# johannes-graeter/limo

Hardware: AMD Instinct MI355X
Metric: keyframe-BA window solves/sec (5 KF, ~2k landmarks) (higher is better)
Workload: dtype f64; 1 GPU; C2: KITTI-00-shaped windows, 5 keyframes x 2000 landmarks, LiDAR depth + ground plane, solveTrimmed schedule {2, trim 5%, <=100 LM iterations}; batch_windows_per_gpu=16384, distinct_windows_per_gpu=4096, observations_per_batch=144288124, depth_observations_per_batch=68405568, parallelism=single, converged=16328

## Files before the change

### limo_amd/csrc/kba_buffers.hpp

```cpp
#pragma once
#include <algorithm>
#include <cstddef>
#include <vector>

#include "kba_pack.hpp"

namespace kba {

template <typename F>
void for_each_buffer(const PackedBatch& P, BatchView& bv, F f) {
    bv.n_win = P.n_win;
    bv.TK = P.TK;
    bv.TL = P.TL;
    bv.TO = P.TO;
    bv.TV = P.TV;
    bv.TG = P.TG;
    bv.n_blk = P.n_blk;
    bv.n_lblk = P.n_lblk;
    bv.n_sblk = P.n_sblk;
    bv.Vmax = P.Vmax;
    bv.SO = P.SO;
    bv.SL = P.SL;
    bv.SG = P.SG;
    bv.SD = P.SD;
// ... 19 lines not shown
    KBA_BUF(lm_c, TL * 3 * D, P.lm.data());
    KBA_BUF(kf_win, TK * I, P.kf_win.data());
    KBA_BUF(kf_blk0, TK * I, P.kf_blk0.data());
    KBA_BUF(kf_nblk, TK * I, P.kf_nblk.data());
    KBA_BUF(kf_gp0, TK * I, P.kf_gp0.data());
    KBA_BUF(kf_ngp, TK * I, P.kf_ngp.data());
    KBA_BUF(cmask, TK * kCamSlots, P.cmask.data());
    KBA_BUF(cpresent, TK * kCamSlots, P.cpresent.data());
    KBA_BUF(cslot, TK * kCamSlots * I, P.cslot.data());
    KBA_BUF(lm_win, TL * I, P.lm_win.data());
    KBA_BUF(lm_id, TL * I, P.lm_id.data());
    KBA_BUF(lm_weight, TL * D, P.lm_weight.data());
    KBA_BUF(lm_state, TL, P.lm_state.data());
    KBA_BUF(lm_gp, TL * I, P.lm_gp.data());
    KBA_BUF(lm_slot, P.lm_slot.size() * I, P.lm_slot.data());
    KBA_BUF(view_kf, TV * I, P.view_kf.data());
    KBA_BUF(view_win, TV * I, P.view_win.data());
    KBA_BUF(view_cam, TV * 16 * D, P.view_cam.data());
    KBA_BUF(view_lin, TV * kViewLin * D, nullptr);
    KBA_BUF(view_lin_c, TV * kViewLin * D, nullptr);
    KBA_BUF(blk_view, NB * I, P.blk_view.data());
    KBA_BUF(blk_obs0, NB * I, P.blk_obs0.data());
    KBA_BUF(blk_n, NB * I, P.blk_n.data());
    KBA_BUF(obs_lm, TO * I, P.obs_lm.data());
    KBA_BUF(obs_u, TO * sizeof(float), P.obs_u.data());
    KBA_BUF(obs_v, TO * sizeof(float), P.obs_v.data());
    KBA_BUF(obs_d, TO * sizeof(float), P.obs_d.data());
    KBA_BUF(lblk_win, NL * I, P.lblk_win.data());
    KBA_BUF(lblk_lm0, NL * I, P.lblk_lm0.data());
    KBA_BUF(lblk_n, NL * I, P.lblk_n.data());
    KBA_BUF(sblk_win, NS * I, P.sblk_win.data());
    KBA_BUF(sblk_lm0, NS * I, P.sblk_lm0.data());
    KBA_BUF(sblk_n, NS * I, P.sblk_n.data());
    KBA_BUF(gp_lm, TG * I, P.gp_lm.data());
    KBA_BUF(gp_kf, TG * I, P.gp_kf.data());
    KBA_BUF(gp_w, TG * D, P.gp_w.data());
    KBA_BUF(gp_r, (size_t)P.SG * D, nullptr);
    KBA_BUF(gp_F, (size_t)P.SG * 10 * D, nullptr);
    KBA_BUF(gp_E, (size_t)P.SG * 3 * D, nullptr);
    KBA_BUF(gp_cost, TG * D, nullptr);
    KBA_BUF(gp_cost_c, TG * D, nullptr);
    KBA_BUF(obs_r, (size_t)(P.evaluate_only ? P.SO * 2 + P.SD : 1) * D, nullptr);
    KBA_BUF(obs_c, (size_t)(P.evaluate_only ? 1 : P.SO * 2) * D, nullptr);
    KBA_BUF(obs_Jp, (size_t)(P.evaluate_only ? P.SO * 12 + P.SD * 6 : 1) * D, nullptr);
    KBA_BUF(obs_Jl, (size_t)(P.evaluate_only ? P.SO * 6 + P.SD * 3 : 1) * D, nullptr);
    if (P.evaluate_only) KBA_BUF(echunk, (size_t)std::max(1, P.n_echunk) * sizeof(EvalChunk), P.echunk.empty() ? nullptr : P.echunk.data());
    KBA_BUF(lv_part, (size_t)(P.lvpart_total > 0 ? P.lvpart_total : 1) * D, nullptr);
    KBA_BUF(lblk_linfail, NL * D, nullptr);
    KBA_BUF(lm_V, (size_t)P.SL * 6 * D, nullptr);
    KBA_BUF(lm_g, (size_t)P.SL * 3 * D, nullptr);
    KBA_BUF(lm_scale, (size_t)P.SL * 3 * D, nullptr);
    KBA_BUF(lm_Li, (size_t)P.SL * 6 * D, nullptr);
    KBA_BUF(lblk_part, NL * 8 * D, nullptr);
    KBA_BUF(Hcc, (size_t)(P.hcc_total > 0 ? P.hcc_total : 1) * D, nullptr);
    KBA_BUF(gc, TK * kCamSlots * D, nullptr);
    KBA_BUF(scale_c, TK * kCamSlots * D, nullptr);
    KBA_BUF(yc, TK * kCamSlots * D, nullptr);
    KBA_BUF(delta_c, TK * kCamSlots * D, nullptr);
    KBA_BUF(S_part, (size_t)(P.spart_total > 0 ? P.spart_total : 1) * D, nullptr);
    KBA_BUF(S_red, (size_t)(P.sred_total > 0 ? P.sred_total : 1) * D, nullptr);
    KBA_BUF(cam_scratch, (size_t)(P.camscr_total > 0 ? P.camscr_total : 1) * D, nullptr);
    KBA_BUF(reg_cost, NW * 2 * D, nullptr);
    KBA_BUF(trim_rep, TL * D, nullptr);
    KBA_BUF(trim_dep, TL * D, nullptr);
    KBA_BUF(n_active, 8 * I, nullptr);
    if (P.n_shards > 1) {
// ... 79 lines not shown
```

### limo_amd/csrc/kba_items.hpp

```cpp
#pragma once
#include "kba_layout.hpp"
#include "kba_lm.hpp"
#include "kba_math.hpp"

#ifndef KBA_SYNC
#define KBA_SYNC() ((void)0)
#endif
#if defined(KBA_PROFILE_TICKS) && defined(__HIPCC__)
__device__ long long kba_ticks[2][24];
#endif
#if defined(KBA_PROFILE_TICKS) && defined(__HIP_DEVICE_COMPILE__)
#define KBA_TICK(n)                                                                   \
    do {                                                                              \
        if (w == 0 && (tid == 0 || tid == nt - 1)) kba_ticks[tid != 0][n] = clock64(); \
    } while (0)
#else
#define KBA_TICK(n) ((void)0)
#endif

namespace kba {

struct LinLane {
    double e[kLinPartial];
    int fail;
};

KBA_HD void view_consts_compute(const double* cam, const double* pose, double* vl);
KBA_HD void view_consts_item(const BatchView& bv, int view) {
    view_consts_compute(bv.view_cam + 16 * (int64_t)view, bv.pose + 7 * (int64_t)bv.view_kf[view], bv.view_lin + (int64_t)kViewLin * view);
}
KBA_HD void view_consts_compute(const double* cam, const double* pose, double* vl) {
    double R[9];
    quat_R(pose, R);
    mat3_mul(cam + 4, R, vl);
    for (int i = 0; i < 3; ++i)
        vl[9 + i] = cam[4 + 3 * i] * pose[4] + cam[4 + 3 * i + 1] * pose[5] + cam[4 + 3 * i + 2] * pose[6] + cam[13 + i];
    for (int i = 0; i < 9; ++i) vl[12 + i] = cam[4 + i];
    for (int i = 0; i < 4; ++i) vl[21 + i] = pose[i];
    vl[25] = cam[0];
    vl[26] = cam[1];
    vl[27] = cam[2];
    const double qq1 = quat_norm2_minus_1(pose);
    for (int i = 0; i < 9; ++i) vl[28 + i] = -2.0 * (R[i] + ((i & 3) == 0 ? qq1 : 0.0));
}

struct LinIn {
    double p[3];
    double w;
    double sw;
    float u, v, d;
    int live;
};

KBA_HD void lin_fetch(const BatchView& bv, int64_t o, int gl, LinIn& in) {
    in.live = bv.lm_state[gl] != 0;
    in.p[0] = bv.lm[3 * (int64_t)gl];
    in.p[1] = bv.lm[3 * (int64_t)gl + 1];
    in.p[2] = bv.lm[3 * (int64_t)gl + 2];
    in.w = bv.lm_weight[gl];
    in.sw = sqrt(in.w);
    in.u = bv.obs_u[o];
    in.v = bv.obs_v[o];
    in.d = bv.obs_d[o];
}

struct CamTmp {
    double G[9], A01[6], v[3], wb, wc, wd;
};
template <class VP>
KBA_HD void lin_cam_half0(VP vl, const double* p, const double* c4, const double* r3, double cost, CamTmp& t, double* out) {
    const double p0 = p[0], p1 = p[1], p2 = p[2];
    const double au = c4[0], sd = c4[3];
    const double a1 = au * c4[1], a2 = au * c4[2];
    const double yv[3] = {vl[28] * p0 + vl[29] * p1 + vl[30] * p2, vl[31] * p0 + vl[32] * p1 + vl[33] * p2, vl[34] * p0 + vl[35] * p1 + vl[36] * p2};
#pragma unroll
    for (int j = 0; j < 3; ++j) {
// ... 480 lines not shown
KBA_HD int schur_need_pad(int nf) { return (schur_need_count(nf) + 31) / 32 * 32; }
KBA_HD void schur_need_decode(int i, int nf, int& ca, int& cb) {
    const int lda = nf + 1;
    ca = (int)(((2 * lda + 1) - sqrt((double)((2 * lda + 1) * (2 * lda + 1) - 8 * i))) * 0.5);
    while (ca > 0 && ca * lda - ca * (ca - 1) / 2 > i) --ca;
    while ((ca + 1) * lda - (ca + 1) * ca / 2 <= i) ++ca;
    cb = ca + (i - (ca * lda - ca * (ca - 1) / 2));
}
KBA_HD int schur_col(int i, int nfq);
KBA_HD int64_t schur_need_offset(int ca, int cb, int nf, int nfq, int nfp) {
    if (cb < nf) return (int64_t)schur_col(ca, nfq) * nfp + schur_col(cb, nfq);
    const int za = schur_col(ca, nfq);
    return za < nfq ? (int64_t)za * nfp + nfq : (int64_t)nfq * nfp + za;
}
KBA_HD void slab_reduce_entry(const BatchView& bv, int w, int n_shards, int i) {
    const WinDesc& wd = bv.win[w];
    const int64_t slab = (int64_t)wd.nf_pad * wd.nf_pad;
    int ca, cb;
    schur_need_decode(i, wd.nf, ca, cb);
    const double* sp = bv.S_part + wd.spart_off + schur_need_offset(ca, cb, wd.nf, wd.nfq, wd.nf_pad);
    double a = 0.0;
    const int q0 = (ca >= wd.nfq || (cb >= wd.nfq && cb < wd.nf)) ? wd.n_sblk_plain : 0;
    for (int q = q0; q < wd.n_sblk; ++q) a += sp[q * slab];
    bv.S_red[wd.sred_off / n_shards + i] = a;
}

KBA_HD int schur_col(int i, int nfq) {
    return i + (i >= nfq ? 1 : 0);
}

KBA_HD int schur_need_index(int n, int ca, int cb) { return ca * (n + 1) - ca * (ca - 1) / 2 + (cb - ca); }
KBA_HD int64_t slab_packed_base(int q, int n_plain, int nf, int nfq) {
    return q < n_plain ? (int64_t)q * schur_need_pad(nfq) : (int64_t)n_plain * schur_need_pad(nfq) + (int64_t)(q - n_plain) * schur_need_pad(nf);
}
KBA_HD int slab_packed_read(bool gp, int ca, int cb, int nf, int nfq) {
    if (gp) return schur_need_index(nf, ca, cb);
    if (ca >= nfq || (cb >= nfq && cb < nf)) return -1;
    return schur_need_index(nfq, ca, cb < nf ? cb : nfq);
}
KBA_HD int slab_packed_write(bool gp, int zr, int zc, int nf, int nfq) {
    const int n = gp ? nf : nfq;
    if (zr > zc || zc > n || (zr == nfq && zc == nfq)) return -1;
    if (zc == nfq) return schur_need_index(n, zr, n);
    if (zr == nfq) return schur_need_index(n, zc - 1, n);
    return schur_need_index(n, zr - (zr > nfq ? 1 : 0), zc - (zc > nfq ? 1 : 0));
}

struct LogProd {
    double m;
    int e;
};
KBA_HD void logprod_mul(LogProd& a, double x) {
    int ex;
    a.m *= frexp(x, &ex);
    a.e += ex;
}
KBA_HD double logprod_log(const LogProd& a) { return log(a.m) + static_cast<double>(a.e) * 0.69314718055994530942; }

KBA_HD void backsub_lane(const BatchView& bv, const SolveConsts& c, int w, int gl, double* part) {
    part[2] = part[3] = part[4] = part[6] = part[7] = 0.0;
    const int state = bv.lm_state[gl];
    const double* xp = bv.lm + 3 * (int64_t)gl;
    const double x[3] = {xp[0], xp[1], xp[2]};
    double xc[3] = {x[0], x[1], x[2]};
    if (state == 0) {
        double* o = bv.lm_c + 3 * (int64_t)gl;
// ... 1211 lines not shown
```

### limo_amd/csrc/kba_kernels.hip

```cpp
#include <hip/hip_runtime.h>

#include <type_traits>

#define KBA_SYNC() __syncthreads()
#include "kba_items.hpp"

namespace kba {

__device__ __forceinline__ double wave_sum(double v) {
#pragma unroll
    for (int off = 32; off > 0; off >>= 1) v += __shfl_down(v, off, 64);
    return v;
}
__device__ __forceinline__ double wave_max(double v) {
#pragma unroll
    for (int off = 32; off > 0; off >>= 1) v = fmax(v, __shfl_down(v, off, 64));
    return v;
}

template <int N>
__device__ __forceinline__ void block_sum(const double* vals, double* lds , double* out_global) {
    const int lane = threadIdx.x & 63, wave = threadIdx.x >> 6;
#pragma unroll
    for (int i = 0; i < N; ++i) {
// ... 594 lines not shown
                }
            }
        }
        __syncthreads();
        const double* zp = Z + (lane >> 4) * ld + (lane & 15);
#pragma unroll
        for (int j = 0; j < NPW; ++j) {
            const int ti = wave + kWideWaves * j;
            if (ti < n_tiles) {
                const int tr = ttr[ti], tc = ttc[ti];
                if (tc < Tt) {
#pragma unroll
                    for (int ks = 0; ks < 12; ++ks)
                        acc[j] = __builtin_amdgcn_mfma_f64_16x16x4f64(zp[ks * 4 * ld + 16 * tr], zp[ks * 4 * ld + 16 * tc], acc[j], 0, 0, 0);
                }
            }
        }
        __syncthreads();
    }
    double* out = bv.S_part + wd.spart_off + (int64_t)schur_slab_of(wd, sb, span, span_gp) * ((int64_t)nfp * nfp);
#pragma unroll
    for (int j = 0; j < NPW; ++j) {
        const int ti = wave + kWideWaves * j;
        if (ti < n_tiles) {
            const int tr = ttr[ti], tc = ttc[ti];
#pragma unroll
            for (int r = 0; r < 4; ++r)
                out[(tr * 16 + (lane >> 4) + 4 * r) * nfp + tc * 16 + (lane & 15)] = acc[j][r];
        }
    }
}

constexpr int kSpBatch = 4;
constexpr int kSpKf = 72;

__host__ __device__ inline int schur_lean_ld(int ncol) { return ncol | 1; }
__host__ __device__ inline int schur_lean_lds_bytes(int ncol) {
    return (3 * kSchurLm * schur_lean_ld(ncol) + 16 + 4 * kSpKf) * (int)sizeof(double) + 4 * 12 * (int)sizeof(int);
}

template <bool COOP>
__device__ __forceinline__ void schur_wave_sync() {
    if constexpr (COOP) {
        __builtin_amdgcn_fence(__ATOMIC_RELEASE, "workgroup");
        __builtin_amdgcn_wave_barrier();
        __builtin_amdgcn_fence(__ATOMIC_ACQUIRE, "workgroup");
    } else {
        __syncthreads();
    }
}
template <int TM, bool GP, bool COOP>
__device__ __forceinline__ void schur_lean_group(const BatchView& bv, int sb, int span, int span_gp, int slab_packed, double* smem) {
    const int w = bv.sblk_win[sb];
    if (!COOP && !bv.st[w].active) return;
    const WinDesc& wd = bv.win[w];
    const int nfq = wd.nfq, nfp = wd.nf_pad;
    const int ncol = GP ? wd.nf + 1 : nfq + 1;
    const int ld = schur_lean_ld(ncol);
    const int Tt = (ncol + 15) / 16;
    constexpr bool kTT = !GP && TM == 2;
    const bool two_tile = kTT && Tt == 2;
    double* Z = smem;
    double* kc = Z + 3 * kSchurLm * ld + 16;
    int* zcs = reinterpret_cast<int*>(kc + 4 * kSpKf);
    const int lane = COOP ? (int)(threadIdx.x & 63) : (int)threadIdx.x, li = lane & 15, kq = lane >> 4;
    const int n_fk = wd.n_fk;
    int my_view = -1, my_kl = -1;
    if (kq < n_fk) {
        my_kl = wd.fk[kq];
        my_view = wd.fk_view[kq];
        double* mine = kc + kq * kSpKf;
        const double* pose = bv.pose + 7 * (int64_t)(wd.kf0 + my_kl);
        if (li == 0) {
            double R[9];
            quat_R(pose, R);
#pragma unroll
            for (int i = 0; i < 9; ++i) mine[i] = R[i];
#pragma unroll
            for (int i = 0; i < 4; ++i) mine[18 + i] = pose[i];
            mine[32] = quat_norm2_minus_1(pose);
        } else if (li < 10) {
            mine[9 + li - 1] = my_view >= 0 ? bv.view_cam[16 * (int64_t)my_view + 4 + li - 1] : 0.0;
        } else if (li == 13) {
            for (int i = 0; i < 12; ++i) mine[59 + i] = my_view >= 0 ? bv.view_lin[(int64_t)kViewLin * my_view + i] : 0.0;
        }
        if (li < kCamSlots) {
            const int slot = wd.cam0 + my_kl * kCamSlots + li;
            mine[22 + li] = bv.scale_c[slot];
            const int ci = bv.cslot[slot];
            zcs[kq * 12 + li] = ci < 0 ? -1 : schur_col(ci, nfq);
        }
    }
    if (lane < 16) Z[3 * kSchurLm * ld + lane] = 0.0;
    schur_wave_sync<COOP>();
    const bool have = kq < n_fk && zcs[kq * 12] >= 0;
    const double* mine = kc + (kq < n_fk ? kq : 0) * kSpKf;
    const int32_t* my_slots = bv.lm_slot + (int64_t)(my_view >= 0 ? my_view - wd.view0 : 0) * bv.SL;
    const int sb_last = schur_group_last(wd, sb, span, span_gp);
    const int lm_first = bv.sblk_lm0[sb];
    const int n_lm_blk = bv.sblk_lm0[sb_last] + bv.sblk_n[sb_last] - lm_first;

    constexpr int NT = (!GP && TM == 2) ? 2 : TM * (TM + 1) / 2;
    v4f64 acc[NT];
#pragma unroll
    for (int i = 0; i < NT; ++i) acc[i] = (v4f64){0.0, 0.0, 0.0, 0.0};

    auto fetch_index = [&](int l0, int& st, int& slot, int& gg) {
        st = 0;
        slot = -1;
        gg = -1;
        if (l0 + li < n_lm_blk) {
            const int gl = lm_first + l0 + li;
            st = bv.lm_state[gl];
            if (have && my_view >= 0) slot = my_slots[gl];
            if (GP && have && st == 1) {
                const int g = bv.lm_gp[gl];
                if (g >= 0 && bv.gp_kf[g] - wd.kf0 == my_kl) gg = g;
            }
        }
    };
    double c4[4], p[3], Bt[6], g3[3], gE[3], gF[kCamSlots];
    bool live = false, seen = false, att = false;
    auto fetch_data = [&](int l0, int st, int slot, int gg) {
        const int gl = lm_first + l0 + li;
        live = st == 1;
        seen = live && slot >= 0;
        att = GP && live && gg >= 0;
        if (seen) {
            c4[0] = bv.obs_c[slot];
            c4[3] = bv.obs_c[bv.SO + slot];
#pragma unroll
            for (int i = 0; i < 3; ++i) p[i] = bv.lm[3 * (int64_t)gl + i];
        }
        const bool want_t = live && (kq == 0 || two_tile);
        if (seen || att || want_t) {
#pragma unroll
            for (int i = 0; i < 6; ++i) Bt[i] = bv.lm_Li[i * bv.SL + gl];
        }
        if (want_t) {
#pragma unroll
            for (int i = 0; i < 3; ++i) g3[i] = bv.lm_g[i * bv.SL + gl];
        }
        if constexpr (GP) {
            if (att) {
#pragma unroll
                for (int i = 0; i < 3; ++i) gE[i] = bv.gp_E[i * bv.SG + gg];
#pragma unroll
                for (int i = 0; i < kCamSlots; ++i) gF[i] = bv.gp_F[i * bv.SG + gg];
            }
        }
    };
    int n_st, n_slot, n_gg;
    {
        int st0, slot0, gg0;
        fetch_index(0, st0, slot0, gg0);
        fetch_index(kSchurLm, n_st, n_slot, n_gg);
        fetch_data(0, st0, slot0, gg0);
    }
    constexpr int NS = GP ? kCamSlots : 6;
    double yt[6] = {0.0, 0.0, 0.0, 0.0, 0.0, 0.0};
    const int mq = li < 8 ? li : li + 8;
    for (int l0 = 0; l0 < n_lm_blk; l0 += kSchurLm) {
        double t3[3] = {0.0, 0.0, 0.0};
        if (live && (kq == 0 || two_tile)) lm_t_of(Bt, g3, t3);
        if (kq == 0 && !two_tile) {
#pragma unroll
            for (int cc = 0; cc < 3; ++cc) Z[(3 * li + cc) * ld + nfq] = live ? t3[cc] : 0.0;
        }
        if (have) {
            double Y[3 * NS];
#pragma unroll
            for (int i = 0; i < 3 * NS; ++i) Y[i] = 0.0;
            if (seen) {
                double M[9], Ft[9];
                rot_tangent_from_R(mine, mine[32], p, M);
                view_xy(mine + 59, p, &c4[1], &c4[2]);
                ft_build(c4, mine + 9, Ft);
                schur_pose_block<true>(Ft, mine, M, Bt, mine + 22, Y);
                if (two_tile) {
#pragma unroll
                    for (int a = 0; a < 6; ++a) yt[a] += Y[a * 3 + 0] * t3[0] + Y[a * 3 + 1] * t3[1] + Y[a * 3 + 2] * t3[2];
                }
            }
            if constexpr (GP) {
                if (att) {
                    const double y0 = gE[0] * Bt[0], y1 = gE[0] * Bt[1] + gE[1] * Bt[2], y2 = gE[0] * Bt[3] + gE[1] * Bt[4] + gE[2] * Bt[5];
#pragma unroll
                    for (int a = 0; a < kCamSlots; ++a) {
                        const double fa = zcs[kq * 12 + a] >= 0 ? gF[a] * mine[22 + a] : 0.0;
                        Y[a * 3 + 0] += fa * y0;
                        Y[a * 3 + 1] += fa * y1;
                        Y[a * 3 + 2] += fa * y2;
                    }
                }
            }
            double* zrow = Z + 3 * li * ld + zcs[kq * 12];
#pragma unroll
            for (int a = 0; a < 6; ++a) {
                zrow[a] = Y[a * 3 + 0];
                zrow[ld + a] = Y[a * 3 + 1];
                zrow[2 * ld + a] = Y[a * 3 + 2];
            }
            if constexpr (GP) {
#pragma unroll
                for (int a = 6; a < kCamSlots; ++a) {
                    const int zc = zcs[kq * 12 + a];
                    if (zc >= 0) {
                        Z[(3 * li + 0) * ld + zc] = Y[a * 3 + 0];
                        Z[(3 * li + 1) * ld + zc] = Y[a * 3 + 1];
                        Z[(3 * li + 2) * ld + zc] = Y[a * 3 + 2];
                    }
                }
            }
        }
        {
            const int st = n_st, slot = n_slot, gg = n_gg;
            fetch_index(l0 + 2 * kSchurLm, n_st, n_slot, n_gg);
            fetch_data(l0 + kSchurLm, st, slot, gg);
        }
        schur_wave_sync<COOP>();
        const double* zp = Z + kq * ld + li;
        if (TM == 1 || Tt == 1) {
#pragma unroll
            for (int h = 0; h < 12; h += kSpBatch) {
                double pa[kSpBatch];
#pragma unroll
                for (int j = 0; j < kSpBatch; ++j) pa[j] = zp[(h + j) * 4 * ld];
#pragma unroll
                for (int j = 0; j < kSpBatch; ++j) acc[0] = __builtin_amdgcn_mfma_f64_16x16x4f64(pa[j], pa[j], acc[0], 0, 0, 0);
            }
        } else if (kTT) {
            if constexpr (kTT) {
                constexpr int kB = 3;
#pragma unroll
                for (int h = 0; h < 12; h += kB) {
                    double pa[kB], pb[kB], pq[kB];
#pragma unroll
                    for (int j = 0; j < kB; ++j) {
                        pa[j] = zp[(h + j) * 4 * ld];
                        pb[j] = zp[(h + j) * 4 * ld + 8];
                        pq[j] = Z[((h + j) * 4 + kq) * ld + mq];
                    }
#pragma unroll
                    for (int j = 0; j < kB; ++j) {
                        acc[0] = __builtin_amdgcn_mfma_f64_16x16x4f64(pa[j], pb[j], acc[0], 0, 0, 0);
                        acc[1] = __builtin_amdgcn_mfma_f64_16x16x4f64(pq[j], pq[j], acc[1], 0, 0, 0);
                    }
                }
            }
        } else if (TM == 2 || Tt == 2) {
// ... 9 lines not shown
                    }
#pragma unroll
                    for (int j = 0; j < kSpBatch; ++j) {
                        acc[0] = __builtin_amdgcn_mfma_f64_16x16x4f64(pa[j], pa[j], acc[0], 0, 0, 0);
                        acc[1] = __builtin_amdgcn_mfma_f64_16x16x4f64(pa[j], pb[j], acc[1], 0, 0, 0);
                        acc[i11] = __builtin_amdgcn_mfma_f64_16x16x4f64(pb[j], pb[j], acc[i11], 0, 0, 0);
                    }
                }
            }
        } else {
            if constexpr (TM >= 3) {
#pragma unroll
                for (int h = 0; h < 12; h += 2) {
                    double pn[2][3];
#pragma unroll
                    for (int j = 0; j < 2; ++j)
#pragma unroll
                        for (int t = 0; t < 3; ++t) pn[j][t] = zp[(h + j) * 4 * ld + 16 * t];
#pragma unroll
                    for (int j = 0; j < 2; ++j) {
                        acc[0] = __builtin_amdgcn_mfma_f64_16x16x4f64(pn[j][0], pn[j][0], acc[0], 0, 0, 0);
                        acc[1] = __builtin_amdgcn_mfma_f64_16x16x4f64(pn[j][0], pn[j][1], acc[1], 0, 0, 0);
                        acc[2] = __builtin_amdgcn_mfma_f64_16x16x4f64(pn[j][0], pn[j][2], acc[2], 0, 0, 0);
                        acc[3] = __builtin_amdgcn_mfma_f64_16x16x4f64(pn[j][1], pn[j][1], acc[3], 0, 0, 0);
                        acc[4] = __builtin_amdgcn_mfma_f64_16x16x4f64(pn[j][1], pn[j][2], acc[4], 0, 0, 0);
                        acc[5] = __builtin_amdgcn_mfma_f64_16x16x4f64(pn[j][2], pn[j][2], acc[5], 0, 0, 0);
                    }
                }
            }
        }
        schur_wave_sync<COOP>();
    }
    const bool packed = !COOP && slab_packed != 0;
    const int q_slab = schur_slab_of(wd, sb, span, span_gp);
    double* out = bv.S_part + wd.spart_off +
                  (packed ? slab_packed_base(q_slab, schur_plain_slabs(wd, span), wd.nf, nfq) : (int64_t)q_slab * ((int64_t)nfp * nfp));
    const int T = nfp / 16;
    if (two_tile && packed) {
#pragma unroll
        for (int r = 0; r < 4; ++r) {
            const int row = kq + 4 * r;
            {
                const int col = 8 + li;
                if (row <= col && col < nfq) out[slab_packed_write(false, row, col, wd.nf, nfq)] = acc[0][r];
            }
            {
                const int a = row < 8 ? row : row + 8, b = mq;
                if (a <= b && b < nfq && !(a < 8 && b >= 16)) out[slab_packed_write(false, a, b, wd.nf, nfq)] = acc[1][r];
            }
        }
        if (have) {
#pragma unroll
            for (int a = 0; a < 6; ++a) {
                double v = yt[a];
                v += __shfl_xor(v, 1, 64);
                v += __shfl_xor(v, 2, 64);
                v += __shfl_xor(v, 4, 64);
                v += __shfl_xor(v, 8, 64);
                if (li == 0) out[slab_packed_write(false, zcs[kq * 12] + a, nfq, wd.nf, nfq)] = v;
            }
        }
        return;
    }
    if (two_tile) {
        double* St = Z;
        for (int i = lane; i < 1024; i += 64) St[i] = 0.0;
        schur_wave_sync<COOP>();
#pragma unroll
        for (int r = 0; r < 4; ++r) {
            const int row = kq + 4 * r;
            {
                const int col = 8 + li;
                if (row <= col && col < nfq) St[row * 32 + col] = acc[0][r];
            }
            {
                const int a = row < 8 ? row : row + 8, b = mq;
                if (a <= b && b < nfq && !(a < 8 && b >= 16)) St[a * 32 + b] = acc[1][r];
            }
        }
        if (have) {
#pragma unroll
            for (int a = 0; a < 6; ++a) {
                double v = yt[a];
                v += __shfl_xor(v, 1, 64);
                v += __shfl_xor(v, 2, 64);
                v += __shfl_xor(v, 4, 64);
                v += __shfl_xor(v, 8, 64);
                if (li == 0) St[(zcs[kq * 12] + a) * 32 + nfq] = v;
            }
        }
        schur_wave_sync<COOP>();
        for (int tc = 0; tc < (T < 2 ? T : 2); ++tc)
            for (int tr = 0; tr <= tc; ++tr) {
#pragma unroll
                for (int r = 0; r < 4; ++r) {
                    const int row = tr * 16 + kq + 4 * r, col = tc * 16 + li;
                    out[row * nfp + col] = St[row * 32 + col];
                }
            }
        return;
    }
    if constexpr (kTT) {
#pragma unroll
        for (int r = 0; r < 4; ++r) {
            const int row = kq + 4 * r, col = li;
            if (packed) {
                const int k = slab_packed_write(false, row, col, wd.nf, nfq);
                if (k >= 0) out[k] = acc[0][r];
            } else {
                out[row * nfp + col] = (row < ncol && col < ncol) ? acc[0][r] : 0.0;
            }
        }
    } else {
        int idx = 0;
#pragma unroll
        for (int tr = 0; tr < TM; ++tr)
#pragma unroll
            for (int tc = tr; tc < TM; ++tc) {
                if (tc < T) {
#pragma unroll
                    for (int r = 0; r < 4; ++r) {
                        const int row = tr * 16 + kq + 4 * r, col = tc * 16 + li;
                        if (packed) {
                            const int k = slab_packed_write(GP, row, col, wd.nf, nfq);
                            if (k >= 0) out[k] = acc[idx][r];
                        } else {
                            out[row * nfp + col] = (row < ncol && col < ncol) ? acc[idx][r] : 0.0;
                        }
                    }
                }
                ++idx;
            }
        if constexpr (GP) {
            if (!packed)
                for (int tc = TM; tc < T; ++tc)
                    for (int tr = 0; tr <= tc; ++tr) {
#pragma unroll
                        for (int r = 0; r < 4; ++r) out[(tr * 16 + kq + 4 * r) * nfp + tc * 16 + li] = 0.0;
                    }
        }
    }
}
template <int TM, bool GP, int WAVES>
__global__ __launch_bounds__(64) __attribute__((amdgpu_waves_per_eu(WAVES, WAVES))) void k_schur_lean(
    BatchView bv, const int32_t* wl, int span, int span_gp, int slab_packed) {
    const int sb = wl_at(bv, wl, blockIdx.x);
    if (sb < 0) return;
    extern __shared__ __attribute__((aligned(16))) double smem[];
    schur_lean_group<TM, GP, false>(bv, sb, span, span_gp, slab_packed, smem);
}

template <int TMP, int TMG>
__global__ __launch_bounds__(64) void k_schur_lean_pair(BatchView bv, const int32_t* wl_plain, int n_plain_cap, const int32_t* wl_gp, int span, int span_gp, int slab_packed) {
    extern __shared__ __attribute__((aligned(16))) double smem[];
    if ((int)blockIdx.x < n_plain_cap) {
        const int sb = wl_at(bv, wl_plain, blockIdx.x);
        if (sb >= 0) schur_lean_group<TMP, false, false>(bv, sb, span, span_gp, slab_packed, smem);
// ... 817 lines not shown
```

### limo_amd/csrc/kba_layout.hpp

```cpp
#pragma once
#include <stddef.h>
#include <stdint.h>

#include "../../include/limo_hip.h"

namespace kba {

constexpr int kMaxKf = 20;
constexpr int kMaxViews = 64;
constexpr int kViewLin = 64;
constexpr int kCamSlots = 10;
constexpr int kMaxNc = kMaxKf * kCamSlots;
constexpr int kBlock = 256;
constexpr int kObsPerLane = 4;
constexpr int kObsBlock = kBlock * kObsPerLane;
constexpr int kSchurLm = 16;
constexpr int kSchurLmPerBlock = 64;
constexpr int kMaxRegRows = 1 + (kMaxKf - 1) * 5 + 3 * kMaxKf;

constexpr int kGpRed = 65;
constexpr int kLinPartial = 28;
constexpr int kLinWaves = 4;

struct EvalChunk {
    int32_t base, view, o0, o1, dep0, pad;
};

struct WinDesc {
    int32_t kf0, n_kf;
    int32_t lm0, n_lm;
    int32_t view0, n_view;
    int32_t obs0, n_obs;
    int32_t blk0, n_blk;
    int32_t lblk0, n_lblk;
    int32_t gp0, n_gp;
    int32_t sblk0, n_sblk;
    int32_t n_sblk_plain;
    int32_t schur_fast, n_fk;
    int32_t fk[4];
    int32_t fk_view[4];
    int32_t nc, nc_pad;
    int32_t nf, nf_pad;
    int32_t nfq;
    int32_t lm_gp0;
    int32_t cam0;
    int32_t reg0;
    int32_t has_scale_reg, has_gp_reg;
    int32_t n_depth, n_repr;
    int32_t do_trim;
    int32_t pose_only;
    int32_t n_view_fixed0;
    int32_t pad_view;
    double scale_w, scale_s0;
    double speed_w, speed_dt, speed_vel[3], speed_Rb[9], speed_tb[3];
    int64_t hcc_off;
    int64_t spart_off;
    int64_t sred_off;
    int64_t xlv_off;
    int64_t lvpart_off;
    int64_t cam_scr_off;
};

struct WinState {
    int32_t active, need_lin, first, accept;
    int32_t iter, max_iter, term, invalid_run;
    int32_t in_phase;
    int32_t compute_scale;
    int32_t n_success, n_unsuccess;
    int32_t acc_solves, acc_iters, acc_success, last_iters;
    int32_t n_trimmed, acc_lin;
    int32_t phase, trim_round;
    int32_t redamp, pad_i;
    double radius, decrease_factor;
    double x_cost, x_norm, fixed_cost;
    double solve_initial_cost, solve_final_cost;
    double first_initial_cost;
    double rho_pending, xnorm_pending, cost_pending;
    double gmax;
};

struct WinRed {
    double lin_cost;
    double gmax;
    double xnorm2;
    double mcc;
    double step2;
    double cand2;
    double cand_cost;
    int32_t lin_fail, chol_fail, cand_fail, pad;
};

enum SchedPhase { PH_IDLE = 0, PH_TRIM_SOLVE = 1, PH_RETRY = 2, PH_TRIM = 3, PH_FINAL = 4, PH_DONE = 5 };

enum SchedList { SL_LBLK = 0, SL_SPLAIN, SL_SFGP, SL_SGEN, SL_WIN, SL_TBLK, SL_TLBLK, SL_TWIN, SL_COUNT };
// ... 22 lines not shown
    WinRed* red;
    double *pose, *pdir, *pdist, *lm;
    double *pose_c, *pdir_c, *pdist_c, *lm_c;
    const int32_t* kf_win;
    const int32_t* kf_blk0;
    const int32_t* kf_nblk;
    const int32_t* kf_gp0;
    const int32_t* kf_ngp;
    uint8_t* cmask;
    uint8_t* cpresent;
    const int32_t* cslot;
    const int32_t* lm_win;
    const int32_t* lm_id;
    const double* lm_weight;
    uint8_t* lm_state;
    const int32_t* lm_gp;
    const int32_t* lm_slot;
    const int32_t* view_kf;
    const int32_t* view_win;
    const double* view_cam;
    double* view_lin_c;
    double* view_lin;
    const int32_t* blk_view;
    const int32_t* blk_obs0;
    const int32_t* blk_n;
    const int32_t* obs_lm;
    const float *obs_u, *obs_v, *obs_d;
    const int32_t* lblk_win;
    const int32_t* lblk_lm0;
    const int32_t* lblk_n;
    const int32_t* sblk_win;
    const int32_t* sblk_lm0;
    const int32_t* sblk_n;
    const int32_t* lblk_owner;
    const int32_t* gp_owner;
    double* x_lv;
    double* x_lf;
    double* x_gp;
    double* x_gc;
    double* x_gcc;
    double* x_lb;
    const double* gp_red;
    int32_t gp_red_P, pad_x;
    const int32_t* gp_lm;
    const int32_t* gp_kf;
    const double* gp_w;
    double *gp_r, *gp_F, *gp_E;
    double* gp_cost;
    double* gp_cost_c;
    double *obs_r, *obs_c;
    double *obs_Jp, *obs_Jl;
    const EvalChunk* echunk;
    int64_t SD;
    int32_t n_echunk, pad_e;
    double* lv_part;
    double* lblk_linfail;
    double *lm_V, *lm_g;
    double *lm_scale;
    double* lm_Li;
    double* lblk_part;
    double *Hcc, *gc;
    double *scale_c, *yc, *delta_c;
    double *S_part;
    double *S_red;
    double* cam_scratch;
    double* reg_cost;
// ... 32 lines not shown
```

### limo_amd/csrc/kba_pack.cpp

```cpp
#include "kba_pack.hpp"

#include <algorithm>
#include <atomic>
#include <chrono>
#include <cmath>
#include <cstdio>
#include <cstdlib>
#include <cstring>
#include <condition_variable>
#include <functional>
#include <limits>
#include <mutex>
#include <numeric>
#include <thread>
#include <pthread.h>
#include <unistd.h>
#include <exception>

#include "kba_items.hpp"

namespace kba {

namespace {
thread_local PackArena* t_pack_arena = nullptr;
// ... 668 lines not shown
            if (P.kf_nblk[k]) P.kf_blk0[k] += bs.blk;
            if (P.kf_ngp[k]) P.kf_gp0[k] += bs.gp;
        }
        for (int l = d.lm0; l < d.lm0 + d.n_lm; ++l)
            if (P.lm_gp[l] >= 0) P.lm_gp[l] += bs.gp;
        auto put = [](auto& dst, const auto& src, int at) { std::copy(src.begin(), src.end(), dst.begin() + at); };
        put(P.blk_view, L.blk_view, bs.blk);
        put(P.blk_obs0, L.blk_obs0, bs.blk);
        put(P.blk_n, L.blk_n, bs.blk);
        put(P.blk_owner, L.blk_owner, bs.blk);
        put(P.lblk_win, L.lblk_win, bs.lblk);
        put(P.lblk_lm0, L.lblk_lm0, bs.lblk);
        put(P.lblk_n, L.lblk_n, bs.lblk);
        put(P.lblk_owner, L.lblk_owner, bs.lblk);
        put(P.sblk_win, L.sblk_win, bs.sblk);
        put(P.sblk_lm0, L.sblk_lm0, bs.sblk);
        put(P.sblk_n, L.sblk_n, bs.sblk);
        put(P.sblk_owner, L.sblk_owner, bs.sblk);
        put(P.gp_lm, L.gp_lm, bs.gp);
        put(P.gp_kf, L.gp_kf, bs.gp);
        put(P.gp_w, L.gp_w, bs.gp);
        put(P.gp_owner, L.gp_owner, bs.gp);
        L = Local();
    });
    if (std::getenv("KBA_PACK_TRACE"))
        std::fprintf(stderr, "[kba] pack: views + sizes %.1f ms, arrays %.1f ms, fill %.1f ms, merge %.1f ms\n", std::chrono::duration<double, std::milli>(t_p0b - t_p0).count(),
                     std::chrono::duration<double, std::milli>(t_p1 - t_p0b).count(), std::chrono::duration<double, std::milli>(t_p2 - t_p1).count(),
                     std::chrono::duration<double, std::milli>(std::chrono::steady_clock::now() - t_p2).count());
    P.TG = (int)P.gp_lm.size();
    P.SG = pad64(std::max(1, P.TG));
    P.n_blk = (int)P.blk_view.size();
    P.n_lblk = (int)P.lblk_win.size();
    P.n_sblk = (int)P.sblk_win.size();
    if (P.evaluate_only) {
        P.echunk.clear();
        P.obs_rank.assign((size_t)std::max(1, P.TO), -1);
        std::vector<int32_t> before((size_t)P.TO + 1, 0);
        for (int o = 0; o < P.TO; ++o) {
            const bool dep = P.obs_d[o] > 0.0f;
            if (dep) P.obs_rank[o] = before[o];
            before[o + 1] = before[o] + (dep ? 1 : 0);
        }
        P.TD = before[P.TO];
        P.SD = pad64(std::max(1, P.TD)) + 64;
        for (int b = 0; b < P.n_blk; ++b) {
            const int o0 = P.blk_obs0[b], o1 = o0 + P.blk_n[b];
            for (int a = o0; a < o1; a += 64) {
                EvalChunk ch;
                ch.base = a;
                ch.view = P.blk_view[b];
                ch.o0 = o0;
                ch.o1 = o1;
                ch.dep0 = before[a];
                ch.pad = 0;
                P.echunk.push_back(ch);
            }
        }
        P.n_echunk = (int)P.echunk.size();
    }
    return LIMO_OK;
}

void run_schedule(Executor& ex, const limo_ba_options& o) {
    using Clock = std::chrono::steady_clock;
    auto run_solve = [&](int max_iter, int select) {
        ex.solve_init(max_iter, select);
// ... 22 lines not shown
```

### limo_amd/csrc/kba_pack.hpp

```cpp
#pragma once
#include <memory>
#include <string>
#include <type_traits>
#include <utility>
#include <vector>

#include "kba_layout.hpp"

namespace kba {

struct PackArena {
    char* base = nullptr;
    size_t cap = 0, used = 0;
    size_t wanted = 0;
};
constexpr size_t kPackArenaMin = 64u << 10;
void pack_arena_lend(PackArena* a);
void pack_arena_register(const void* base, size_t cap, bool add);
bool pack_arena_owns(const void* p);
void* pack_arena_take(size_t bytes);
struct PackArenaLend {
    explicit PackArenaLend(PackArena* a) { pack_arena_lend(a); }
    ~PackArenaLend() { pack_arena_lend(nullptr); }
    PackArenaLend(const PackArenaLend&) = delete;
// ... 28 lines not shown
template <typename T>
using uvec = std::vector<T, default_init_allocator<T>>;

struct PackedBatch {
    int32_t n_win = 0, TK = 0, TL = 0, TO = 0, TV = 0, TG = 0, n_blk = 0, n_lblk = 0, n_sblk = 0, Vmax = 0;
    int64_t SO = 0, SL = 0, SG = 0;
    int64_t SD = 0;
    int32_t TD = 0;
    int64_t hcc_total = 0, spart_total = 0, sred_total = 0, camscr_total = 0, lvpart_total = 0, xlv_total = 0;
    bool evaluate_only = false;
    int32_t n_shards = 1;
    std::vector<int32_t> blk_owner, lblk_owner, sblk_owner, gp_owner;
    std::vector<WinDesc> win;
    std::vector<double> pose, pdir, pdist;
    uvec<double> lm;
    std::vector<int32_t> kf_win, kf_blk0, kf_nblk, kf_gp0, kf_ngp;
    std::vector<uint8_t> cmask, cpresent;
    std::vector<int32_t> cslot;
    uvec<int32_t> lm_gp;
    uvec<int32_t> lm_win, lm_slot;
    uvec<int32_t> lm_id;
    uvec<double> lm_weight;
    uvec<uint8_t> lm_state;
    std::vector<int32_t> view_kf, view_win;
    std::vector<double> view_cam;
    std::vector<int32_t> blk_view, blk_obs0, blk_n;
    std::vector<EvalChunk> echunk;
    int32_t n_echunk = 0;
    std::vector<int32_t> obs_rank;
    uvec<int32_t> obs_lm;
    uvec<float> obs_u, obs_v, obs_d;
    uvec<int32_t> obs_src;
    std::vector<int32_t> lblk_win, lblk_lm0, lblk_n, sblk_win, sblk_lm0, sblk_n;
    std::vector<int32_t> gp_lm, gp_kf;
    std::vector<double> gp_w;
};

struct PackOptions {
    bool pose_only = false;
    bool evaluate_only = false;
    const limo_speed_prior* prior = nullptr;
    int shards = 1;
};

int pack_windows(int32_t n, const limo_ba_window* windows, const limo_ba_options& opts, const PackOptions& po,
                 PackedBatch& out, std::string& err);

SolveConsts make_consts(const limo_ba_options& o);

struct Executor {
    virtual ~Executor() {}
    virtual void solve_init(int max_iter, int select) = 0;
    virtual void linearize() = 0;
    virtual int active_count() = 0;
    virtual void step() = 0;
    virtual void trim() = 0;
    virtual void expire(int) {}
};

void run_schedule(Executor& ex, const limo_ba_options& o);

}
```

### limo_amd/csrc/limo_hip.hip

```cpp
#include <hip/hip_runtime.h>
#include <rccl/rccl.h>

#include <algorithm>
#include <chrono>
#include <cmath>
#include <cstdio>
#include <cstring>
#include <atomic>
#include <memory>
#include <new>
#include <string>
#include <thread>
#include <vector>

#include "kba_kernels.hip"

#include "kba_batch_plan.hpp"
#include "kba_buffers.hpp"
#include "kba_rows.hpp"

using namespace kba;

#include "limo_ctx.hpp"

// ... 277 lines not shown
        return LIMO_OK;
    }

    bool spart_has_packed = false;
    bool pristine = true;
    int reset_state() {
        pristine = true;
        HIP_TRY(ctx, hipMemcpyAsync(bv.st, st0.data(), sizeof(WinState) * st0.size(), hipMemcpyHostToDevice, ctx->stream));
        HIP_TRY(ctx, hipMemcpyAsync(bv.pose, d_pose0, sizeof(double) * 7 * P.TK, hipMemcpyDeviceToDevice, ctx->stream));
        HIP_TRY(ctx, hipMemcpyAsync(bv.pdir, d_pdir0, sizeof(double) * 3 * P.TK, hipMemcpyDeviceToDevice, ctx->stream));
        HIP_TRY(ctx, hipMemcpyAsync(bv.pdist, d_pdist0, sizeof(double) * P.TK, hipMemcpyDeviceToDevice, ctx->stream));
        HIP_TRY(ctx, hipMemcpyAsync(bv.lm, d_lm0, sizeof(double) * 3 * P.TL, hipMemcpyDeviceToDevice, ctx->stream));
        HIP_TRY(ctx, hipMemcpyAsync(bv.lm_state, d_lm_state0, P.TL, hipMemcpyDeviceToDevice, ctx->stream));
        return LIMO_OK;
    }

    void note(hipError_t e, const char* what) {
        if (e != hipSuccess && rc == LIMO_OK) {
            rc = LIMO_ERR_RUNTIME;
            ctx->err = std::string(what) + ": " + hipGetErrorString(e);
        }
    }
    void note_nccl(ncclResult_t r, const char* what) {
        if (r != ncclSuccess && rc == LIMO_OK) {
            rc = LIMO_ERR_RUNTIME;
            ctx->err = std::string(what) + ": " + ncclGetErrorString(r);
        }
    }
#define LAUNCH_CHECK(what) note(hipGetLastError(), what)

    SolveConsts consts_for(const limo_ba_options& o) const {
        SolveConsts k = make_consts(o);
        const bool sharded = shard_P > 1;
        k.schur_span = sharded ? 1 : 2;
        k.schur_span_gp = 1;
        k.schur_nslab = sharded ? shard_P : 0;
        k.schur_packed = sharded ? 1 : 0;
        k.slab_packed = sharded ? 0 : 1;
        return k;
    }

    void exchange(int point) {
        if (shard_P == 1) return;
        hipStream_t s = ctx->stream;
        size_t off, count;
        xl.range(point, off, count);
        for (size_t i = 0; i < pv.size(); ++i) {
            if (shard_virtual) {
                hipLaunchKernelGGL(k_unpack, dim3(cdiv((int64_t)count, 256)), dim3(256), 0, s, xl, (const WinDesc*)d_win_orig, (const double*)(blocks[i] + off), arena_c,
                                   local_shards[i], (int64_t)off, (int64_t)count);
                LAUNCH_CHECK("k_unpack");
            } else {
                if (ctx->xfn) {
                    host_exchange(blocks[i] + off, d_gather, count, 0);
                } else {
                    note_nccl(ncclAllGather(blocks[i] + off, d_gather, count, ncclDouble, (ncclComm_t)ctx->comm, s), "ncclAllGather");
                }
                for (int q = 0; q < ctx->comm_world; ++q) {
                    hipLaunchKernelGGL(k_unpack, dim3(cdiv((int64_t)count, 256)), dim3(256), 0, s, xl, (const WinDesc*)d_win_orig,
                                       (const double*)(d_gather + (size_t)q * count), arena_c, (int)i * ctx->comm_world + q, (int64_t)off, (int64_t)count);
                    LAUNCH_CHECK("k_unpack");
                }
            }
            ++n_exchanges;
            exchange_bytes += (int64_t)count * (int64_t)sizeof(double);
        }
    }
    void host_exchange(const double* src, double* dst, size_t count, int kind) {
// ... 1234 lines not shown
```

Measured before the change: 37100 windows/s.

## Precompute per-group Schur descriptors and reuse view rotation in lean Schur kernel

Adds a 128-byte SchurGroup record per Schur block, built at pack time, holding the window index, landmark range, keyframe/view/column mappings and output offsets. The lean Schur kernel loads this single record instead of chasing WinDesc, sblk arrays and cslot. It also stores the rotation and quaternion norm term alongside view_lin, so the kernel reads them instead of recomputing quat_R per group. Index loads are split into issue/mask phases so they can be issued ahead of the active check. In exchange the kernel reads view_lin beyond the old 37 slots, which depends on kViewLin having room, and the per-keyframe shared-memory record shrinks from 72 to 41 doubles.

```diff
diff --git a/limo_amd/csrc/kba_buffers.hpp b/limo_amd/csrc/kba_buffers.hpp
--- a/limo_amd/csrc/kba_buffers.hpp
+++ b/limo_amd/csrc/kba_buffers.hpp
@@ -75,6 +75,7 @@
     KBA_BUF(sblk_win, NS * I, P.sblk_win.data());
     KBA_BUF(sblk_lm0, NS * I, P.sblk_lm0.data());
     KBA_BUF(sblk_n, NS * I, P.sblk_n.data());
+    KBA_BUF(sgrp, NS * sizeof(SchurGroup), P.sgrp.empty() ? nullptr : P.sgrp.data());
     KBA_BUF(gp_lm, TG * I, P.gp_lm.data());
     KBA_BUF(gp_kf, TG * I, P.gp_kf.data());
     KBA_BUF(gp_w, TG * D, P.gp_w.data());
diff --git a/limo_amd/csrc/kba_items.hpp b/limo_amd/csrc/kba_items.hpp
--- a/limo_amd/csrc/kba_items.hpp
+++ b/limo_amd/csrc/kba_items.hpp
@@ -25,11 +25,13 @@
     int fail;
 };
 
-KBA_HD void view_consts_compute(const double* cam, const double* pose, double* vl);
+constexpr int kViewLinRot = 37;
+KBA_HD void view_consts_compute(const double* cam, const double* pose, double* vl, double* rot = nullptr);
 KBA_HD void view_consts_item(const BatchView& bv, int view) {
-    view_consts_compute(bv.view_cam + 16 * (int64_t)view, bv.pose + 7 * (int64_t)bv.view_kf[view], bv.view_lin + (int64_t)kViewLin * view);
-}
-KBA_HD void view_consts_compute(const double* cam, const double* pose, double* vl) {
+    double* vl = bv.view_lin + (int64_t)kViewLin * view;
+    view_consts_compute(bv.view_cam + 16 * (int64_t)view, bv.pose + 7 * (int64_t)bv.view_kf[view], vl, vl + kViewLinRot);
+}
+KBA_HD void view_consts_compute(const double* cam, const double* pose, double* vl, double* rot) {
     double R[9];
     quat_R(pose, R);
     mat3_mul(cam + 4, R, vl);
@@ -42,6 +44,10 @@
     vl[27] = cam[2];
     const double qq1 = quat_norm2_minus_1(pose);
     for (int i = 0; i < 9; ++i) vl[28 + i] = -2.0 * (R[i] + ((i & 3) == 0 ? qq1 : 0.0));
+    if (rot) {
+        for (int i = 0; i < 9; ++i) rot[i] = R[i];
+        rot[9] = qq1;
+    }
 }
 
 struct LinIn {
@@ -588,6 +594,30 @@
 KBA_HD int schur_need_index(int n, int ca, int cb) { return ca * (n + 1) - ca * (ca - 1) / 2 + (cb - ca); }
 KBA_HD int64_t slab_packed_base(int q, int n_plain, int nf, int nfq) {
     return q < n_plain ? (int64_t)q * schur_need_pad(nfq) : (int64_t)n_plain * schur_need_pad(nfq) + (int64_t)(q - n_plain) * schur_need_pad(nf);
+}
+KBA_HD SchurGroup schur_group_make(const WinDesc& wd, int w, int sb, int span, int span_gp, const int32_t* sblk_lm0, const int32_t* sblk_n,
+                                   const int32_t* cslot) {
+    SchurGroup g;
+    const int sb_last = schur_group_last(wd, sb, span, span_gp);
+    g.w = w;
+    g.lm_first = sblk_lm0[sb];
+    g.n_lm = sblk_lm0[sb_last] + sblk_n[sb_last] - g.lm_first;
+    g.n_fk = wd.n_fk;
+    g.nf = wd.nf, g.nfq = wd.nfq, g.nf_pad = wd.nf_pad;
+    g.kf0 = wd.kf0, g.view0 = wd.view0, g.cam0 = wd.cam0;
+    g.q_slab = schur_slab_of(wd, sb, span, span_gp);
+    g.pad = 0;
+    for (int k = 0; k < 4; ++k) {
+        const bool on = k < wd.n_fk;
+        g.kl[k] = on ? wd.fk[k] : -1;
+        g.view[k] = on ? wd.fk_view[k] : -1;
+        const int ci = on ? cslot[wd.cam0 + wd.fk[k] * kCamSlots] : -1;
+        g.col0[k] = ci < 0 ? -1 : schur_col(ci, wd.nfq);
+        g.pad2[k] = 0;
+    }
+    g.off_tile = wd.spart_off + (int64_t)g.q_slab * ((int64_t)wd.nf_pad * wd.nf_pad);
+    g.off_packed = wd.spart_off + slab_packed_base(g.q_slab, schur_plain_slabs(wd, span), wd.nf, wd.nfq);
+    return g;
 }
 KBA_HD int slab_packed_read(bool gp, int ca, int cb, int nf, int nfq) {
     if (gp) return schur_need_index(nf, ca, cb);
diff --git a/limo_amd/csrc/kba_kernels.hip b/limo_amd/csrc/kba_kernels.hip
--- a/limo_amd/csrc/kba_kernels.hip
+++ b/limo_amd/csrc/kba_kernels.hip
@@ -650,7 +650,8 @@
 }
 
 constexpr int kSpBatch = 4;
-constexpr int kSpKf = 72;
+constexpr int kSpKf = 41;
+constexpr int kSpRc = 9, kSpScale = 18, kSpQq1 = 28, kSpH = 29;
 
 __host__ __device__ inline int schur_lean_ld(int ncol) { return ncol | 1; }
 __host__ __device__ inline int schur_lean_lds_bytes(int ncol) {
@@ -669,11 +670,16 @@
 }
 template <int TM, bool GP, bool COOP>
 __device__ __forceinline__ void schur_lean_group(const BatchView& bv, int sb, int span, int span_gp, int slab_packed, double* smem) {
-    const int w = bv.sblk_win[sb];
-    if (!COOP && !bv.st[w].active) return;
-    const WinDesc& wd = bv.win[w];
-    const int nfq = wd.nfq, nfp = wd.nf_pad;
-    const int ncol = GP ? wd.nf + 1 : nfq + 1;
+    SchurGroup g;
+    if (span == kSchurSpan && span_gp == kSchurSpanGp) {
+        g = bv.sgrp[sb];
+    } else {
+        const int w = bv.sblk_win[sb];
+        g = schur_group_make(bv.win[w], w, sb, span, span_gp, bv.sblk_lm0, bv.sblk_n, bv.cslot);
+    }
+    const int active = COOP ? 1 : __hip_atomic_load(&bv.st[g.w].active, __ATOMIC_RELAXED, __HIP_MEMORY_SCOPE_AGENT);
+    const int nfq = g.nfq, nfp = g.nf_pad;
+    const int ncol = GP ? g.nf + 1 : nfq + 1;
     const int ld = schur_lean_ld(ncol);
     const int Tt = (ncol + 15) / 16;
     constexpr bool kTT = !GP && TM == 2;
@@ -682,60 +688,37 @@
     double* kc = Z + 3 * kSchurLm * ld + 16;
     int* zcs = reinterpret_cast<int*>(kc + 4 * kSpKf);
     const int lane = COOP ? (int)(threadIdx.x & 63) : (int)threadIdx.x, li = lane & 15, kq = lane >> 4;
-    const int n_fk = wd.n_fk;
-    int my_view = -1, my_kl = -1;
-    if (kq < n_fk) {
-        my_kl = wd.fk[kq];
-        my_view = wd.fk_view[kq];
-        double* mine = kc + kq * kSpKf;
-        const double* pose = bv.pose + 7 * (int64_t)(wd.kf0 + my_kl);
-        if (li == 0) {
-            double R[9];
-            quat_R(pose, R);
-#pragma unroll
-            for (int i = 0; i < 9; ++i) mine[i] = R[i];
-#pragma unroll
-            for (int i = 0; i < 4; ++i) mine[18 + i] = pose[i];
-            mine[32] = quat_norm2_minus_1(pose);
-        } else if (li < 10) {
-            mine[9 + li - 1] = my_view >= 0 ? bv.view_cam[16 * (int64_t)my_view + 4 + li - 1] : 0.0;
-        } else if (li == 13) {
-            for (int i = 0; i < 12; ++i) mine[59 + i] = my_view >= 0 ? bv.view_lin[(int64_t)kViewLin * my_view + i] : 0.0;
-        }
-        if (li < kCamSlots) {
-            const int slot = wd.cam0 + my_kl * kCamSlots + li;
-            mine[22 + li] = bv.scale_c[slot];
-            const int ci = bv.cslot[slot];
-            zcs[kq * 12 + li] = ci < 0 ? -1 : schur_col(ci, nfq);
-        }
-    }
-    if (lane < 16) Z[3 * kSchurLm * ld + lane] = 0.0;
-    schur_wave_sync<COOP>();
-    const bool have = kq < n_fk && zcs[kq * 12] >= 0;
-    const double* mine = kc + (kq < n_fk ? kq : 0) * kSpKf;
-    const int32_t* my_slots = bv.lm_slot + (int64_t)(my_view >= 0 ? my_view - wd.view0 : 0) * bv.SL;
-    const int sb_last = schur_group_last(wd, sb, span, span_gp);
-    const int lm_first = bv.sblk_lm0[sb];
-    const int n_lm_blk = bv.sblk_lm0[sb_last] + bv.sblk_n[sb_last] - lm_first;
+    const int n_fk = g.n_fk;
+    const int my_kl = kq == 0 ? g.kl[0] : kq == 1 ? g.kl[1] : kq == 2 ? g.kl[2] : g.kl[3];
+    const int my_view = kq == 0 ? g.view[0] : kq == 1 ? g.view[1] : kq == 2 ? g.view[2] : g.view[3];
+    const int my_col0 = kq == 0 ? g.col0[0] : kq == 1 ? g.col0[1] : kq == 2 ? g.col0[2] : g.col0[3];
+    const bool have = my_col0 >= 0;
+    const int slot0 = g.cam0 + (my_kl >= 0 ? my_kl : 0) * kCamSlots;
+    const int32_t* my_slots = bv.lm_slot + (int64_t)(my_view >= 0 ? my_view - g.view0 : 0) * bv.SL;
+    const int lm_first = g.lm_first, n_lm_blk = g.n_lm;
 
     constexpr int NT = (!GP && TM == 2) ? 2 : TM * (TM + 1) / 2;
     v4f64 acc[NT];
 #pragma unroll
     for (int i = 0; i < NT; ++i) acc[i] = (v4f64){0.0, 0.0, 0.0, 0.0};
 
-    auto fetch_index = [&](int l0, int& st, int& slot, int& gg) {
-        st = 0;
-        slot = -1;
-        gg = -1;
-        if (l0 + li < n_lm_blk) {
-            const int gl = lm_first + l0 + li;
-            st = bv.lm_state[gl];
-            if (have && my_view >= 0) slot = my_slots[gl];
-            if (GP && have && st == 1) {
-                const int g = bv.lm_gp[gl];
-                if (g >= 0 && bv.gp_kf[g] - wd.kf0 == my_kl) gg = g;
-            }
-        }
+    auto index_issue = [&](int l0, int& st, int& slot, int& gr) {
+        const int i = l0 + li < n_lm_blk ? l0 + li : n_lm_blk - 1;
+        const int gl = lm_first + i;
+        st = bv.lm_state[gl];
+        slot = my_slots[gl];
+        gr = -1;
+        if constexpr (GP) gr = bv.lm_gp[gl];
+    };
+    auto index_kf = [&](int gr) {
+        if constexpr (GP) return bv.gp_kf[gr >= 0 ? gr : 0];
+        return 0;
+    };
+    auto index_mask = [&](int l0, int& st, int& slot, int& gg, int kf) {
+        const bool in = l0 + li < n_lm_blk;
+        st = in ? st : 0;
+        slot = in && have && my_view >= 0 ? slot : -1;
+        gg = GP && in && have && st == 1 && gg >= 0 && kf - g.kf0 == my_kl ? gg : -1;
     };
     double c4[4], p[3], Bt[6], g3[3], gE[3], gF[kCamSlots];
     bool live = false, seen = false, att = false;
@@ -768,13 +751,36 @@
             }
         }
     };
-    int n_st, n_slot, n_gg;
+    int n_st, n_slot, n_gg, n_kf;
     {
-        int st0, slot0, gg0;
-        fetch_index(0, st0, slot0, gg0);
-        fetch_index(kSchurLm, n_st, n_slot, n_gg);
-        fetch_data(0, st0, slot0, gg0);
-    }
+        int st0, sl0, gg0;
+        index_issue(0, st0, sl0, gg0);
+        index_issue(kSchurLm, n_st, n_slot, n_gg);
+        const double* vl = bv.view_lin + (int64_t)kViewLin * (my_view >= 0 ? my_view : 0);
+        const double v0 = vl[li], v1 = vl[16 + li], v2 = vl[32 + li];
+        const int my_slot = slot0 + (li < kCamSlots ? li : 0);
+        const double sc = bv.scale_c[my_slot];
+        const int ci = bv.cslot[my_slot];
+        const int kf_0 = index_kf(gg0);
+        n_kf = index_kf(n_gg);
+        index_mask(0, st0, sl0, gg0, kf_0);
+        fetch_data(0, st0, sl0, gg0);
+        if (!active) return;
+        if (kq < n_fk) {
+            double* mine_w = kc + kq * kSpKf;
+            const bool vw = my_view >= 0;
+            mine_w[li < 12 ? kSpH + li : kSpRc + li - 12] = vw ? v0 : 0.0;
+            if (li < 5) mine_w[kSpRc + 4 + li] = vw ? v1 : 0.0;
+            if (li >= 5 && li < 15) mine_w[li == 14 ? kSpQq1 : li - 5] = vw ? v2 : 0.0;
+            if (li < kCamSlots) {
+                mine_w[kSpScale + li] = sc;
+                zcs[kq * 12 + li] = ci < 0 ? -1 : schur_col(ci, nfq);
+            }
+        }
+        if (lane < 16) Z[3 * kSchurLm * ld + lane] = 0.0;
+        schur_wave_sync<COOP>();
+    }
+    const double* mine = kc + (kq < n_fk ? kq : 0) * kSpKf;
     constexpr int NS = GP ? kCamSlots : 6;
     double yt[6] = {0.0, 0.0, 0.0, 0.0, 0.0, 0.0};
     const int mq = li < 8 ? li : li + 8;
@@ -791,10 +797,10 @@
             for (int i = 0; i < 3 * NS; ++i) Y[i] = 0.0;
             if (seen) {
                 double M[9], Ft[9];
-                rot_tangent_from_R(mine, mine[32], p, M);
-                view_xy(mine + 59, p, &c4[1], &c4[2]);
-                ft_build(c4, mine + 9, Ft);
-                schur_pose_block<true>(Ft, mine, M, Bt, mine + 22, Y);
+                rot_tangent_from_R(mine, mine[kSpQq1], p, M);
+                view_xy(mine + kSpH, p, &c4[1], &c4[2]);
+                ft_build(c4, mine + kSpRc, Ft);
+                schur_pose_block<true>(Ft, mine, M, Bt, mine + kSpScale, Y);
                 if (two_tile) {
 #pragma unroll
                     for (int a = 0; a < 6; ++a) yt[a] += Y[a * 3 + 0] * t3[0] + Y[a * 3 + 1] * t3[1] + Y[a * 3 + 2] * t3[2];
@@ -805,7 +811,7 @@
                     const double y0 = gE[0] * Bt[0], y1 = gE[0] * Bt[1] + gE[1] * Bt[2], y2 = gE[0] * Bt[3] + gE[1] * Bt[4] + gE[2] * Bt[5];
 #pragma unroll
                     for (int a = 0; a < kCamSlots; ++a) {
-                        const double fa = zcs[kq * 12 + a] >= 0 ? gF[a] * mine[22 + a] : 0.0;
+                        const double fa = zcs[kq * 12 + a] >= 0 ? gF[a] * mine[kSpScale + a] : 0.0;
                         Y[a * 3 + 0] += fa * y0;
                         Y[a * 3 + 1] += fa * y1;
                         Y[a * 3 + 2] += fa * y2;
@@ -832,8 +838,10 @@
             }
         }
         {
-            const int st = n_st, slot = n_slot, gg = n_gg;
-            fetch_index(l0 + 2 * kSchurLm, n_st, n_slot, n_gg);
+            int st = n_st, slot = n_slot, gg = n_gg;
+            index_mask(l0 + kSchurLm, st, slot, gg, n_kf);
+            index_issue(l0 + 2 * kSchurLm, n_st, n_slot, n_gg);
+            n_kf = index_kf(n_gg);
             fetch_data(l0 + kSchurLm, st, slot, gg);
         }
         schur_wave_sync<COOP>();
@@ -909,9 +917,7 @@
         schur_wave_sync<COOP>();
     }
     const bool packed = !COOP && slab_packed != 0;
-    const int q_slab = schur_slab_of(wd, sb, span, span_gp);
-    double* out = bv.S_part + wd.spart_off +
-                  (packed ? slab_packed_base(q_slab, schur_plain_slabs(wd, span), wd.nf, nfq) : (int64_t)q_slab * ((int64_t)nfp * nfp));
+    double* out = bv.S_part + (packed ? g.off_packed : g.off_tile);
     const int T = nfp / 16;
     if (two_tile && packed) {
 #pragma unroll
@@ -919,11 +925,11 @@
             const int row = kq + 4 * r;
             {
                 const int col = 8 + li;
-                if (row <= col && col < nfq) out[slab_packed_write(false, row, col, wd.nf, nfq)] = acc[0][r];
+                if (row <= col && col < nfq) out[slab_packed_write(false, row, col, g.nf, nfq)] = acc[0][r];
             }
             {
                 const int a = row < 8 ? row : row + 8, b = mq;
-                if (a <= b && b < nfq && !(a < 8 && b >= 16)) out[slab_packed_write(false, a, b, wd.nf, nfq)] = acc[1][r];
+                if (a <= b && b < nfq && !(a < 8 && b >= 16)) out[slab_packed_write(false, a, b, g.nf, nfq)] = acc[1][r];
             }
         }
         if (have) {
@@ -934,7 +940,7 @@
                 v += __shfl_xor(v, 2, 64);
                 v += __shfl_xor(v, 4, 64);
                 v += __shfl_xor(v, 8, 64);
-                if (li == 0) out[slab_packed_write(false, zcs[kq * 12] + a, nfq, wd.nf, nfq)] = v;
+                if (li == 0) out[slab_packed_write(false, zcs[kq * 12] + a, nfq, g.nf, nfq)] = v;
             }
         }
         return;
@@ -982,7 +988,7 @@
         for (int r = 0; r < 4; ++r) {
             const int row = kq + 4 * r, col = li;
             if (packed) {
-                const int k = slab_packed_write(false, row, col, wd.nf, nfq);
+                const int k = slab_packed_write(false, row, col, g.nf, nfq);
                 if (k >= 0) out[k] = acc[0][r];
             } else {
                 out[row * nfp + col] = (row < ncol && col < ncol) ? acc[0][r] : 0.0;
@@ -999,7 +1005,7 @@
                     for (int r = 0; r < 4; ++r) {
                         const int row = tr * 16 + kq + 4 * r, col = tc * 16 + li;
                         if (packed) {
-                            const int k = slab_packed_write(GP, row, col, wd.nf, nfq);
+                            const int k = slab_packed_write(GP, row, col, g.nf, nfq);
                             if (k >= 0) out[k] = acc[idx][r];
                         } else {
                             out[row * nfp + col] = (row < ncol && col < ncol) ? acc[idx][r] : 0.0;
diff --git a/limo_amd/csrc/kba_layout.hpp b/limo_amd/csrc/kba_layout.hpp
--- a/limo_amd/csrc/kba_layout.hpp
+++ b/limo_amd/csrc/kba_layout.hpp
@@ -16,6 +16,7 @@
 constexpr int kObsBlock = kBlock * kObsPerLane;
 constexpr int kSchurLm = 16;
 constexpr int kSchurLmPerBlock = 64;
+constexpr int kSchurSpan = 2, kSchurSpanGp = 1;
 constexpr int kMaxRegRows = 1 + (kMaxKf - 1) * 5 + 3 * kMaxKf;
 
 constexpr int kGpRed = 65;
@@ -60,6 +61,23 @@
     int64_t lvpart_off;
     int64_t cam_scr_off;
 };
+
+struct alignas(128) SchurGroup {
+    int32_t w;
+    int32_t lm_first, n_lm;
+    int32_t n_fk;
+    int32_t nf, nfq, nf_pad;
+    int32_t kf0, view0, cam0;
+    int32_t q_slab;
+    int32_t pad;
+    int32_t kl[4];
+    int32_t view[4];
+    int32_t col0[4];
+    int64_t off_tile;
+    int64_t off_packed;
+    int32_t pad2[4];
+};
+static_assert(sizeof(SchurGroup) == 128, "one cache line per record");
 
 struct WinState {
     int32_t active, need_lin, first, accept;
@@ -148,6 +166,7 @@
     const int32_t* sblk_win;
     const int32_t* sblk_lm0;
     const int32_t* sblk_n;
+    const SchurGroup* sgrp;
     const int32_t* lblk_owner;
     const int32_t* gp_owner;
     double* x_lv;
diff --git a/limo_amd/csrc/kba_pack.cpp b/limo_amd/csrc/kba_pack.cpp
--- a/limo_amd/csrc/kba_pack.cpp
+++ b/limo_amd/csrc/kba_pack.cpp
@@ -724,6 +724,13 @@
     P.n_blk = (int)P.blk_view.size();
     P.n_lblk = (int)P.lblk_win.size();
     P.n_sblk = (int)P.sblk_win.size();
+    P.sgrp.assign((size_t)P.n_sblk, SchurGroup{});
+    for_windows([&](int w) {
+        const WinDesc& d = P.win[w];
+        if (!d.schur_fast) return;
+        for (int sb = d.sblk0; sb < d.sblk0 + d.n_sblk; ++sb)
+            P.sgrp[sb] = schur_group_make(d, w, sb, kSchurSpan, kSchurSpanGp, P.sblk_lm0.data(), P.sblk_n.data(), P.cslot.data());
+    });
     if (P.evaluate_only) {
         P.echunk.clear();
         P.obs_rank.assign((size_t)std::max(1, P.TO), -1);
diff --git a/limo_amd/csrc/kba_pack.hpp b/limo_amd/csrc/kba_pack.hpp
--- a/limo_amd/csrc/kba_pack.hpp
+++ b/limo_amd/csrc/kba_pack.hpp
@@ -84,6 +84,7 @@
     uvec<float> obs_u, obs_v, obs_d;
     uvec<int32_t> obs_src;
     std::vector<int32_t> lblk_win, lblk_lm0, lblk_n, sblk_win, sblk_lm0, sblk_n;
+    std::vector<SchurGroup> sgrp;
     std::vector<int32_t> gp_lm, gp_kf;
     std::vector<double> gp_w;
 };
diff --git a/limo_amd/csrc/limo_hip.hip b/limo_amd/csrc/limo_hip.hip
--- a/limo_amd/csrc/limo_hip.hip
+++ b/limo_amd/csrc/limo_hip.hip
@@ -333,8 +333,8 @@
     SolveConsts consts_for(const limo_ba_options& o) const {
         SolveConsts k = make_consts(o);
         const bool sharded = shard_P > 1;
-        k.schur_span = sharded ? 1 : 2;
-        k.schur_span_gp = 1;
+        k.schur_span = sharded ? 1 : kSchurSpan;
+        k.schur_span_gp = kSchurSpanGp;
         k.schur_nslab = sharded ? shard_P : 0;
         k.schur_packed = sharded ? 1 : 0;
         k.slab_packed = sharded ? 0 : 1;
```

Measured after the change: 37670 windows/s, median of 6. 1.5% higher.
